# neo-sonar/neo-dsp

Hardware: AMD Instinct MI355X
Metric: Msamples/sec UPOLS convolver (block=512, IR=10s@48k); achieved HBM GB/s (higher is better)
Workload: dtype f32; 1 GPU; UPOLS c5full: 2048 channels in all, 2048 on rank 0 of 1 GPU(s) (split over the ranks), B=512, L=480000 taps (P=938), one block per step; channels_per_gpu=2048, channels_total=2048, block=512, taps=480000, partitions=938, far_group=3, step_group=4, far_form=transform, stored spectra, parallelism=channel-shard x1 (no collective)

## Files before the change

### neo-dsp_amd/csrc/upols_levels.hip

```cpp
#include "upols_device.hpp"
#include "upols_handle.hpp"

#include <algorithm>
#include <chrono>
#include <cmath>
#include <cstring>
#include <type_traits>
#include <vector>

namespace neo_hip {

#ifdef NEO_TIMELINE
#define NEO_TL_MARK(a)                                                                                 \
    do {                                                                                               \
        if (threadIdx.x == 0 && (a).tl)                                                                \
            static_cast<unsigned long long*>((a).tl)[4 * int64_t(blockIdx.x) + 3] = wall_clock64();    \
    } while (0)
#else
#define NEO_TL_MARK(a) \
    do {               \
    } while (0)
#endif
#ifdef NEO_PS_PROBE
#define NEO_PS_MARK(a, i)                                                                              \
// ... 282 lines not shown
        cmac(yb, h0b, xb, false);
        X[k0] = k0 == 0 ? c2r_join_w<B>(cf{ya.x, 0.f}, cf{ya.y, 0.f}, cf{1.f, 0.f}, 0)
                        : c2r_join_w<B>(ya, yb, cf{wa.x, -wa.y}, k0);
        X[k1] = c2r_join_w<B>(yb, k0 == 0 ? yb : ya, cf{wb.x, -wb.y}, k1);
    }
    __syncthreads();
    NEO_PS_MARK(a, 4);
    if (tid < 64) c2r_tail<B, OLA, EW, true, true, WT>(X, fft, tw, a.out + int64_t(c) * a.ld_out, prev_c, tid);
    NEO_PS_MARK(a, 5);
}

__device__ __forceinline__ __amdgpu_buffer_rsrc_t buf_rsrc(const void* p, int64_t bytes)
{
    return __builtin_amdgcn_make_buffer_rsrc(const_cast<void*>(p), 0, int(bytes), 0x00020000);
}

__device__ __forceinline__ cf buf_ld(__amdgpu_buffer_rsrc_t r, int voff, int soff)
{
    return __builtin_bit_cast(cf, __builtin_amdgcn_raw_buffer_load_b64(r, voff, soff, 2 ));
}

__device__ __forceinline__ void buf_st(cf v, __amdgpu_buffer_rsrc_t r, int voff, int soff)
{
    typedef unsigned u2v __attribute__((ext_vector_type(2)));
    __builtin_amdgcn_raw_buffer_store_b64(__builtin_bit_cast(u2v, v), r, voff, soff, 0);
}

#ifndef NEO_H_POLICY
#define NEO_H_POLICY 0
#endif
__device__ __forceinline__ cf ld_h(const cf* p, int band_end)
{
    if (NEO_H_POLICY && band_end <= 64) return *p;
    return ld_nt(p);
}

template<int D>
__device__ __forceinline__ float xor_sum(float v)
{
    const unsigned u = __float_as_uint(v);
    if constexpr (D == 16) {
        const auto r = __builtin_amdgcn_permlane16_swap(u, u, false, false);
        return __uint_as_float(r[0]) + __uint_as_float(r[1]);
    } else {
        static_assert(D == 32, "lane distance 16 or 32");
        const auto r = __builtin_amdgcn_permlane32_swap(u, u, false, false);
        return __uint_as_float(r[0]) + __uint_as_float(r[1]);
    }
}

template<int T, int NPL, int NPG, int JH>
__device__ __forceinline__ void toep_role(const slice_args& sa, const toep_arg& ta, int bid, char* smem)
{
    static_assert((NPG == 1 || NPG == 4 || NPG == 8 || NPG == 16) && T % JH == 0, "toeplitz slice geometry");
    constexpr int TJ = T / JH, LPU = 16 * NPG, UPW = 256 / LPU, WPU = NPG < 4 ? 1 : NPG / 4, NX = NPL + TJ - 1;
    f2v* red = reinterpret_cast<f2v*>(smem);
    const int t = threadIdx.x, col = t & 15, pg = (t >> 4) % NPG, us = t / LPU;
    const int wu = pg >> 2, q4 = pg & 3;
    const int gpc = sa.B / 16;
    int wb = bid;
    if constexpr (JH == 2 && UPW == 1) {
        if (bid < ta.nwg / 16 * 16) {
            const int r = bid & 15;
            wb = (bid & ~15) + (r & 7) * 2 + (r >> 3);
        }
    }
    const int u = ta.u0 + wb * UPW + us;
    const bool live = u < ta.u1;
    const int uc = live ? u : ta.u1 - 1;
    const int jh = uc % JH, cg = uc / JH, c = cg / gpc, k = (cg - c * gpc) * 16 + col;
    const int j0 = jh * TJ, pa = ta.a + pg * NPL;
    f2v acc[TJ];
#pragma unroll
    for (int j = 0; j < TJ; ++j) acc[j] = f2v(0.f);
    if constexpr (UPW == 1) {
        const int cu = __builtin_amdgcn_readfirstlane(c);
        const int ps8 = int(sa.pstride * int(sizeof(cf)));
        const __amdgpu_buffer_rsrc_t hres = buf_rsrc(sa.H + int64_t(cu) * sa.cstride, int64_t(ta.b) * ps8);
        const __amdgpu_buffer_rsrc_t xres = buf_rsrc(sa.fdl + int64_t(cu) * sa.cstride, int64_t(sa.ring) * ps8);
        if (live && pa < ta.b) {
            cf xr[NX], hm[NPL];
            int r0 = ta.tw + j0 + TJ - 1 - pa - (NX - 1);
            r0 = r0 < 0 ? r0 + sa.ring : r0;
            const int dw = sa.ring - r0;
            const int v0 = r0 * ps8 + k * int(sizeof(cf)), vw = v0 - sa.ring * ps8;
#pragma unroll
            for (int i = 0; i < NX; ++i) {
                const int d = NX - 1 - i;
                xr[i] = buf_ld(xres, (d >= dw ? vw : v0) + d * ps8, 0);
            }
            const int hv0 = pa * ps8 + k * int(sizeof(cf));
#pragma unroll
            for (int m = 0; m < NPL; ++m) hm[m] = buf_ld(hres, hv0, m * ps8);
#pragma unroll
            for (int m = 0; m < NPL; ++m) {
                const pk_coef h(hm[m], k == 0);
#pragma unroll
                for (int jj = 0; jj < TJ; ++jj) h.mac(acc[jj], xr[TJ - 1 - jj + m]);
            }
        }
    } else {
        const cf* Hc = sa.H + int64_t(c) * sa.cstride + k;
        const cf* Xc = sa.fdl + int64_t(c) * sa.cstride + k;
        if (live && pa < ta.b) {
            cf xr[NX], hm[NPL];
#pragma unroll
            for (int i = 0; i < NX; ++i) {
                int r = ta.tw + j0 + TJ - 1 - pa - i;
                r = r < 0 ? r + sa.ring : r;
                xr[i] = ld_nt(Xc + int64_t(r) * sa.pstride);
            }
#pragma unroll
            for (int m = 0; m < NPL; ++m) hm[m] = pa + m < ta.b ? ld_h(Hc + int64_t(pa + m) * sa.pstride, ta.b) : cf{0.f, 0.f};
#pragma unroll
            for (int m = 0; m < NPL; ++m) {
                const pk_coef h(hm[m], k == 0);
#pragma unroll
                for (int jj = 0; jj < TJ; ++jj) h.mac(acc[jj], xr[TJ - 1 - jj + m]);
            }
        }
    }
    if constexpr (NPG >= 4) {
#pragma unroll
        for (int j = 0; j < TJ; ++j) {
            acc[j].x = xor_sum<16>(acc[j].x);
            acc[j].y = xor_sum<16>(acc[j].y);
            acc[j].x = xor_sum<32>(acc[j].x);
            acc[j].y = xor_sum<32>(acc[j].y);
        }
    }
    if constexpr (WPU > 1) {
        if (wu > 0 && q4 == 0) {
#pragma unroll
            for (int j = 0; j < TJ; ++j) red[((us * (WPU - 1) + wu - 1) * TJ + j) * 16 + col] = acc[j];
        }
        __syncthreads();
    }
    if (wu == 0 && q4 == 0 && live) {
        cf* o = ta.slab + int64_t(c) * ta.cs + int64_t(j0) * sa.B + k;
#pragma unroll
        for (int j = 0; j < TJ; ++j) {
            f2v v = acc[j];
            if constexpr (WPU > 1) {
#pragma unroll
                for (int w = 1; w < WPU; ++w) v += red[((us * (WPU - 1) + w - 1) * TJ + j) * 16 + col];
            }
            o[int64_t(j) * sa.B] = cf{v.x, v.y};
        }
    }
}

__device__ __forceinline__ void cmac_pk(f2v& acc, cf h, cf x)
{
    const f2v xv = {x.x, x.y};
    acc = __builtin_elementwise_fma(f2v{h.x, h.x}, xv, acc);
    acc = __builtin_elementwise_fma(f2v{-h.y, h.y}, xv.yx, acc);
}

template<bool BIN0>
__device__ __forceinline__ void t32_step(f2v (&acc)[4], cf (&xw)[4], cf h, cf xn, bool z0)
{
    xw[3] = xw[2];
    xw[2] = xw[1];
    xw[1] = xw[0];
    xw[0] = xn;
    if constexpr (BIN0) {
        const pk_coef hk(h, z0);
#pragma unroll
        for (int o = 0; o < 4; ++o) hk.mac(acc[o], xw[o]);
    } else {
#pragma unroll
        for (int o = 0; o < 4; ++o) cmac_pk(acc[o], h, xw[o]);
    }
}

template<bool BIN0>
__device__ __forceinline__ void t32_walk(const cf* hc, const cf* xc, int ib, int m0, int m1, bool z0, f2v (&acc)[4])
{
    constexpr int KP = 4;
    cf xw[4];
#pragma unroll
    for (int o = 0; o < 3; ++o) xw[o] = xc[ib - m0 + 1 + o];
    int m = m0;
    for (; m + 2 * KP <= m1; m += 2 * KP) {
        float4 h2[KP], x2[KP];
#pragma unroll
        for (int i = 0; i < KP; ++i) {
            h2[i] = *reinterpret_cast<const float4*>(hc + m + 2 * i);
            x2[i] = *reinterpret_cast<const float4*>(xc + ib - (m + 2 * i) - 1);
        }
#pragma unroll
        for (int i = 0; i < KP; ++i) {
            t32_step<BIN0>(acc, xw, cf{h2[i].x, h2[i].y}, cf{x2[i].z, x2[i].w}, z0);
            t32_step<BIN0>(acc, xw, cf{h2[i].z, h2[i].w}, cf{x2[i].x, x2[i].y}, z0);
        }
    }
    for (; m < m1; ++m) t32_step<BIN0>(acc, xw, hc[m], xc[ib - m], z0);
}

template<int T, int NB, int JH>
struct toep_tile {
    static constexpr int UPW = 32 / T, LPU = 256 / UPW, NQ = LPU / 16;
    static constexpr int TP = T / JH, QUADS = TP / 4, NG = NQ / QUADS;
    static constexpr int HS = NB + 2, XS = NB + TP + 2;
    static constexpr int NH = (NB + NQ - 1) / NQ, NXL = (NB + TP - 1 + NQ - 1) / NQ;
    static constexpr int LDS = UPW * 16 * (HS + XS) * int(sizeof(cf));
    static_assert(NG >= 2 && NQ % QUADS == 0 && TP % 4 == 0, "toeplitz tile geometry");
};

template<int T, int NB, int JH>
__device__ __forceinline__ void toep_lds_role(const slice_args& sa, const toep_arg& ta, int bid, char* smem)
{
    using G = toep_tile<T, NB, JH>;
    static_assert(G::LDS <= kSliceLds, "toeplitz tile");
    const int t = threadIdx.x, us = t / G::LPU, lt = t % G::LPU, col = lt & 15, q = lt >> 4;
    cf* hs = reinterpret_cast<cf*>(smem) + us * 16 * (G::HS + G::XS);
    cf* xs = hs + 16 * G::HS;
    const int u = ta.u0 + bid * G::UPW + us, gpc = sa.B / 16;
    const bool live = u < ta.u1;
    const int uc = live ? u : ta.u1 - 1, jp = uc % JH, cg = uc / JH, c = cg / gpc, g = cg - c * gpc;
    const int k = g * 16 + col, nb = ta.b - ta.a, nx = nb + G::TP - 1, R = sa.ring, jpart = jp * G::TP;
    int rb = ta.tw + jpart - (ta.b - 1);
    rb = rb < 0 ? rb + R : rb;
    cf hv[G::NH], xv[G::NXL];
    if constexpr (G::UPW == 1) {
        const int cu = __builtin_amdgcn_readfirstlane(c), ps8 = int(sa.pstride * int(sizeof(cf)));
        const __amdgpu_buffer_rsrc_t hres = buf_rsrc(sa.H + int64_t(cu) * sa.cstride, int64_t(ta.b) * ps8);
        const __amdgpu_buffer_rsrc_t xres = buf_rsrc(sa.fdl + int64_t(cu) * sa.cstride, int64_t(R) * ps8);
#pragma unroll
        for (int i = 0; i < G::NH; ++i) {
            const int m = q + G::NQ * i;
            if (m < nb) hv[i] = buf_ld(hres, (ta.a + m) * ps8 + k * int(sizeof(cf)), 0);
        }
#pragma unroll
        for (int i = 0; i < G::NXL; ++i) {
            const int r = q + G::NQ * i;
            if (r < nx) xv[i] = buf_ld(xres, (rb + r >= R ? rb + r - R : rb + r) * ps8 + k * int(sizeof(cf)), 0);
        }
    } else {
        const cf* Hc = sa.H + int64_t(c) * sa.cstride + k;
        const cf* Xc = sa.fdl + int64_t(c) * sa.cstride + k;
#pragma unroll
        for (int i = 0; i < G::NH; ++i) {
            const int m = q + G::NQ * i;
            if (live && m < nb) hv[i] = ld_h(Hc + int64_t(ta.a + m) * sa.pstride, ta.b);
        }
#pragma unroll
        for (int i = 0; i < G::NXL; ++i) {
            const int r = q + G::NQ * i;
            if (live && r < nx) xv[i] = ld_nt(Xc + int64_t(rb + r >= R ? rb + r - R : rb + r) * sa.pstride);
        }
    }
    const int odd = nb & 1;
    if (live) {
#pragma unroll
        for (int i = 0; i < G::NH; ++i)
            if (q + G::NQ * i < nb) hs[col * G::HS + q + G::NQ * i] = hv[i];
#pragma unroll
        for (int i = 0; i < G::NXL; ++i)
            if (q + G::NQ * i < nx) xs[col * G::XS + odd + q + G::NQ * i] = xv[i];
    }
    __syncthreads();
    NEO_TL_MARK(sa);
    const int grp = q / G::QUADS, j0 = 4 * (q - grp * G::QUADS), nq = ((nb + G::NG - 1) / G::NG + 1) & ~1;
    const int m0 = grp * nq < nb ? grp * nq : nb, m1 = m0 + nq < nb ? m0 + nq : nb;
    f2v acc[4] = {f2v(0.f), f2v(0.f), f2v(0.f), f2v(0.f)};
    const cf* hc = hs + col * G::HS;
    const cf* xc = xs + col * G::XS + odd;
    if (live && m0 < m1) {
        if (g == 0) t32_walk<true>(hc, xc, j0 + nb - 1, m0, m1, col == 0, acc);
        else t32_walk<false>(hc, xc, j0 + nb - 1, m0, m1, false, acc);
    }
    __syncthreads();
    constexpr int LG = 16 * G::QUADS;
    f2v* red = reinterpret_cast<f2v*>(smem);
    const int lg = lt - grp * LG;
    if (grp) {
#pragma unroll
        for (int o = 0; o < 4; ++o) red[((us * (G::NG - 1) + grp - 1) * LG + lg) * 4 + o] = acc[o];
    }
    __syncthreads();
    if (!grp && live) {
        cf* o = ta.slab + int64_t(c) * ta.cs + int64_t(jpart + j0) * sa.B + k;
#pragma unroll
        for (int i = 0; i < 4; ++i) {
            f2v v = acc[i];
#pragma unroll
            for (int r = 1; r < G::NG; ++r) v += red[((us * (G::NG - 1) + r - 1) * LG + lg) * 4 + i];
            o[int64_t(i) * sa.B] = cf{v.x, v.y};
        }
    }
}

constexpr int kBigJH = 8, kBigJP = kBigT / kBigJH, kBigNC = 192;
constexpr int kBigHS = kBigNC + 2, kBigXS = kBigNC + kBigJP + 2;
static_assert(16 * (kBigHS + kBigXS) * int(sizeof(cf)) <= kSliceLds, "big level tile");

__device__ __forceinline__ void toep_big_role(const slice_args& sa, const toep_arg& ta, int bid, char* smem)
{
    constexpr int NH = kBigNC / 16, NXL = (kBigNC + kBigJP - 1 + 15) / 16;
    cf* hs = reinterpret_cast<cf*>(smem);
    cf* xs = hs + 16 * kBigHS;
    const int t = threadIdx.x, col = t & 15, qq = t >> 4, quad = qq & 3, quarter = qq >> 2;
    int wb = bid;
    if (bid < ta.nwg / 64 * 64) {
        const int r = bid & 63;
        wb = (bid & ~63) + (r & 7) * 8 + (r >> 3);
    }
    const int u = ta.u0 + wb, jp = u % kBigJH, cg = u / kBigJH, gpc = sa.B / 16;
    const int c = __builtin_amdgcn_readfirstlane(cg / gpc), g = __builtin_amdgcn_readfirstlane(cg - (cg / gpc) * gpc);
    const int k = g * 16 + col, nb = ta.b - ta.a, R = sa.ring, jpart = jp * kBigJP;
    const int ps8 = int(sa.pstride * int(sizeof(cf)));
    const __amdgpu_buffer_rsrc_t hres = buf_rsrc(sa.H + int64_t(c) * sa.cstride, int64_t(ta.b) * ps8);
    const __amdgpu_buffer_rsrc_t xres = buf_rsrc(sa.fdl + int64_t(c) * sa.cstride, int64_t(R) * ps8);
    f2v acc[4] = {f2v(0.f), f2v(0.f), f2v(0.f), f2v(0.f)};
    for (int mc = 0; mc < nb; mc += kBigNC) {
        const int nc = nb - mc < kBigNC ? nb - mc : kBigNC, nx = nc + kBigJP - 1;
        int rb = (ta.tw + jpart - (ta.a + mc + nc - 1)) % R;
        rb = rb < 0 ? rb + R : rb;
        cf hv[NH], xv[NXL];
#pragma unroll
        for (int i = 0; i < NH; ++i) {
            const int m = qq + 16 * i;
            if (m < nc) hv[i] = buf_ld(hres, (ta.a + mc + m) * ps8 + k * int(sizeof(cf)), 0);
        }
#pragma unroll
        for (int i = 0; i < NXL; ++i) {
            const int r = qq + 16 * i;
            if (r < nx) xv[i] = buf_ld(xres, (rb + r >= R ? rb + r - R : rb + r) * ps8 + k * int(sizeof(cf)), 0);
        }
        if (mc) __syncthreads();
        const int odd = nc & 1;
#pragma unroll
        for (int i = 0; i < NH; ++i)
            if (qq + 16 * i < nc) hs[col * kBigHS + qq + 16 * i] = hv[i];
#pragma unroll
        for (int i = 0; i < NXL; ++i)
            if (qq + 16 * i < nx) xs[col * kBigXS + odd + qq + 16 * i] = xv[i];
        __syncthreads();
        const int nq = ((nc + 3) / 4 + 1) & ~1, m0 = quarter * nq, m1 = m0 + nq < nc ? m0 + nq : nc;
        if (m0 < m1) {
            const cf* hc = hs + col * kBigHS;
            const cf* xc = xs + col * kBigXS + odd;
            if (g == 0) t32_walk<true>(hc, xc, nc - 1 + 4 * quad, m0, m1, col == 0, acc);
            else t32_walk<false>(hc, xc, nc - 1 + 4 * quad, m0, m1, false, acc);
        }
    }
    __syncthreads();
    f2v* red = reinterpret_cast<f2v*>(smem);
    const int ql = t & 63;
    if (quarter) {
#pragma unroll
        for (int o = 0; o < 4; ++o) red[((quarter - 1) * 64 + ql) * 4 + o] = acc[o];
    }
    __syncthreads();
    if (!quarter) {
        cf* o = ta.slab + int64_t(c) * ta.cs + int64_t(jpart + 4 * quad) * sa.B + k;
#pragma unroll
        for (int i = 0; i < 4; ++i) {
            const f2v v = acc[i] + red[ql * 4 + i] + red[(64 + ql) * 4 + i] + red[(128 + ql) * 4 + i];
            o[int64_t(i) * sa.B] = cf{v.x, v.y};
        }
    }
}


__device__ __forceinline__ cf pack_bin0(cf zf, cf zm, int f)
{
    if (f == 0 || f == kFN / 2) return zf;
    if (f < kFN / 2) return cscale(cadd(zf, cconj(zm)), 0.5f);
    const cf d = csub(zm, cconj(zf));
    return cf{0.5f * d.y, -0.5f * d.x};
}

__device__ __forceinline__ cf unpack_bin0(cf wf, cf wm, int f)
{
    if (f == 0 || f == kFN / 2) return wf;
    const cf dc = f < kFN / 2 ? wf : cconj(wm);
    const cf ny = f < kFN / 2 ? wm : cconj(wf);
    return cf{dc.x - ny.y, dc.y + ny.x};
}

template<bool PACK>
__device__ __forceinline__ void bin0_exchange(cf (&v)[16], cf* z, int a, int cp)
{
    if (cp == 0) {
#pragma unroll
        for (int i = 0; i < 16; ++i) z[a + 16 * i] = v[i];
    }
    __syncthreads();
    if (cp == 0) {
#pragma unroll
        for (int i = 0; i < 16; ++i) {
            const int f = a + 16 * i;
            const cf m = z[(kFN - f) & (kFN - 1)];
            v[i] = PACK ? pack_bin0(v[i], m, f) : unpack_bin0(v[i], m, f);
        }
    }
}

constexpr int kF1UG = 4;
constexpr int kFarKMax = 4;

__host__ __device__ __forceinline__ int far_first(int c, int K) { return 1 + ((c - 1) % K + K) % K; }

template<int FPL, int K>
__device__ __forceinline__ void far1_mac(const slice_args& sa, int u, int f0, int col)
{
    constexpr int NS = 16 / FPL;
    static_assert(NS >= K - 1 || K == 1, "history of the previous round");
    const int gpc = sa.B / 16, c = u / gpc, g = u - c * gpc, k = g * 16 + col;
    const int M = sa.M, nseg = sa.nseg, wn = sa.f1wn;
    auto slot = [&](int s) { return ((wn - s - 1) % M + M) % M; };
    const int64_t fs = sa.B, sp = int64_t(kFN) * fs;
    const int s0 = sa.fnfresh < nseg ? sa.fnfresh : nseg;
    const cf* hc = sa.hf + int64_t(c) * sa.fsc + int64_t(f0) * fs + k;
    const cf* xc = sa.xf + int64_t(c) * sa.fsc + int64_t(f0) * fs + k;
    f2v acc[K][FPL];
    cf xp[K > 1 ? K - 1 : 1][FPL];
    bool z0[FPL];
#pragma unroll
    for (int j = 0; j < FPL; ++j) {
#pragma unroll
        for (int w = 0; w < K; ++w) acc[w][j] = f2v(0.f);
        z0[j] = g == 0 && col == 0 && ((f0 + 4 * j) & (kFN / 2 - 1)) == 0;
    }
    for (int sb = s0; sb < nseg; sb += NS) {
        cf xv[NS][FPL], hv[NS][FPL];
#pragma unroll
        for (int i = 0; i < NS; ++i) {
            if (sb + i < nseg) {
                const cf* hs = hc + (sb + i) * sp;
                const cf* xs = xc + slot(sb + i) * sp;
#pragma unroll
                for (int j = 0; j < FPL; ++j) {
                    hv[i][j] = ld_nt(hs + 4 * j * fs);
                    xv[i][j] = ld_nt(xs + 4 * j * fs);
                }
            }
        }
#pragma unroll
        for (int i = 0; i < NS; ++i) {
            if (sb + i < nseg) {
#pragma unroll
                for (int j = 0; j < FPL; ++j) {
                    const pk_coef h(hv[i][j], z0[j]);
#pragma unroll
                    for (int w = 0; w < K; ++w)
                        if (sb + i - w >= s0) h.mac(acc[w][j], i >= w ? xv[i - w][j] : xp[w - i - 1][j]);
                }
            }
        }
        if constexpr (K > 1) {
#pragma unroll
            for (int d = 0; d < K - 1; ++d)
#pragma unroll
                for (int j = 0; j < FPL; ++j) xp[d][j] = xv[NS - 1 - d][j];
        }
    }
#pragma unroll
    for (int w = 0; w < K; ++w) {
        cf* o = sa.f1acc + (int64_t(((wn + w) % sa.fK) * sa.fU + u) * kFN + f0) * 16 + col;
#pragma unroll
        for (int j = 0; j < FPL; ++j) o[4 * j * 16] = cf{acc[w][j].x, acc[w][j].y};
    }
}

template<int FPL, int KMAX>
__device__ __forceinline__ void far1_role(const slice_args& sa, int bid)
{
    constexpr int FR = 4 * FPL, PPG = kFN / FR;
    const int t = threadIdx.x, cl = t & 63, fq = t >> 6;
    const int grp = bid / PPG, part = bid - grp * PPG;
    const int g4 = sa.f1g0 + grp * sa.f1gs;
    const int u = g4 * kF1UG + (cl >> 4);
    if (u < sa.f1u0 || u >= sa.f1u1) return;
    const int f0 = part * FR + fq;
    const int K = sa.fK, cls = sa.f1mode ? g4 % K : 0;
    if (sa.f1mode == 0 || (cls != sa.f1cls && far_first(cls, K) > sa.f1wn)) {
        far1_mac<FPL, 1>(sa, u, f0, cl & 15);
    } else if (cls == sa.f1cls) {
        if constexpr (KMAX <= 2) {
            far1_mac<FPL, 2>(sa, u, f0, cl & 15);
        } else {
            if (K == 2) far1_mac<FPL, 2>(sa, u, f0, cl & 15);
            else if (K == 3) far1_mac<FPL, 3>(sa, u, f0, cl & 15);
            else far1_mac<FPL, kFarKMax>(sa, u, f0, cl & 15);
        }
    }
}

__device__ __forceinline__ void far2a_role(const slice_args& sa, int bid, char* smem)
{
    cf* lds = reinterpret_cast<cf*>(smem);
    cf* z = lds + 16 * 16 * 16;
    cf* tws = z + kFN;
    const int t = threadIdx.x, a = t >> 4, cp = t & 15;
    const int gpc = sa.B / 16, u = sa.f2u0 + bid, c = u / gpc, g = u - c * gpc, k = g * 16 + cp;
// ... 230 lines not shown
        if (unit0) bin0_exchange<true>(hv, z, a, cp);
#pragma unroll
        for (int i = 0; i < 16; ++i) pk_coef(hv[i], z0(i)).mac(acc[i], x[i]);
    }
    cf v[16];
#pragma unroll
    for (int i = 0; i < 16; ++i) v[i] = cf{acc[i].x, acc[i].y};
    __syncthreads();
    NEO_TL_MARK(sa);
    if (unit0) bin0_exchange<false>(v, z, a, cp);
    col_fft<1, 16>(v, lds, tws, a, cp, true);
    constexpr float sc = 1.0f / kFN;
    const __amdgpu_buffer_rsrc_t ores = buf_rsrc(sa.f3ff + int64_t(c) * sa.fcs, int(kFN * fs * int(sizeof(cf))) / 2);
    const int vo = int((int64_t(a) * fs + k) * int(sizeof(cf)));
#pragma unroll
    for (int m = 8; m < 16; ++m)
        buf_st(cscale(v[m], sc), ores, vo, int(16 * (m - 8) * fs * int(sizeof(cf))));
}

struct off_args {
    const cf* fdl;
    const cf* hf;
    const cf* twf;
    cf* y;
    int64_t cstride, pstride;
    int64_t hcs;
    int ring, B, nseg, w;
};

#ifndef NEO_OFF_PF
#define NEO_OFF_PF 0
#endif
template<int WP>
__global__ __launch_bounds__(256) __attribute__((amdgpu_waves_per_eu(WP == 1 ? 3 : 2))) void k_off_mac(off_args sa)
{
    __shared__ cf lds[16 * 16 * 16];
    __shared__ cf z[kFN];
    __shared__ cf tws[kFN];
    __shared__ cf xh[8 * 256];
    const int t = threadIdx.x, a = t >> 4, cp = t & 15;
    const int gpc = sa.B / 16, u = blockIdx.x, c = u / gpc, g = u - c * gpc, k = g * 16 + cp;
    const bool unit0 = g == 0;
    const int64_t fs = sa.B;
    const int spec = int(int64_t(kFN) * fs * int(sizeof(cf)));
    tws[t] = sa.twf[t];
    const __amdgpu_buffer_rsrc_t fres =
        buf_rsrc(sa.fdl + int64_t(c) * sa.cstride, int64_t(sa.ring) * sa.pstride * int(sizeof(cf)));
    const __amdgpu_buffer_rsrc_t hres = buf_rsrc(sa.hf + int64_t(c) * sa.hcs, int64_t(sa.nseg) * spec);
    const int ps8 = int(sa.pstride * int(sizeof(cf))), ko = k * int(sizeof(cf));
    const int vo = int((int64_t(a) * fs + k) * int(sizeof(cf)));
    auto z0 = [&](int i) { return unit0 && cp == 0 && ((a + 16 * i) & (kFN / 2 - 1)) == 0; };
    auto row = [&](int r) { return r >= sa.ring ? r - sa.ring : r; };
    f2v acc[WP][16];
#pragma unroll
    for (int w = 0; w < WP; ++w)
#pragma unroll
        for (int i = 0; i < 16; ++i) acc[w][i] = f2v(0.f);
    int r0 = (sa.w + kFarT * (WP - 2) + a) % sa.ring;
    r0 = r0 < 0 ? r0 + sa.ring : r0;
    cf xp[WP > 1 ? 16 : 1];
    cf nx[NEO_OFF_PF >= 1 ? 8 : 1], nh[NEO_OFF_PF >= 2 ? 16 : 1];
    auto load_rows = [&](cf* dst, int n0, int n1) {
#pragma unroll
        for (int n = n0; n < n1; ++n) dst[n - n0] = buf_ld(fres, row(r0 + 16 * n) * ps8 + ko, 0);
    };
    auto load_spec = [&](cf* dst, int q) {
#pragma unroll
        for (int i = 0; i < 16; ++i) dst[i] = buf_ld(hres, vo, q * spec + int(16 * i * fs * int(sizeof(cf))));
    };
    __syncthreads();
    for (int q = 1 - WP; q < sa.nseg; ++q) {
        cf x[16], hv[16];
        if (q == 1 - WP) {
            load_rows(x, 0, 16);
        } else {
            if constexpr (NEO_OFF_PF >= 1) {
#pragma unroll
                for (int n = 0; n < 8; ++n) x[n] = nx[n];
            } else {
                load_rows(x, 0, 8);
            }
#pragma unroll
            for (int n = 8; n < 16; ++n) x[n] = xh[(n - 8) * 256 + t];
        }
        if (q >= 0) {
            if constexpr (NEO_OFF_PF >= 2) {
                if (q == 0) load_spec(hv, 0);
                else {
#pragma unroll
                    for (int i = 0; i < 16; ++i) hv[i] = nh[i];
                }
            } else {
                load_spec(hv, q);
            }
        }
#pragma unroll
        for (int n = 0; n < 8; ++n) xh[n * 256 + t] = x[n];
        r0 = r0 - kFarT < 0 ? r0 - kFarT + sa.ring : r0 - kFarT;
        if constexpr (NEO_OFF_PF >= 1)
            if (q + 1 < sa.nseg) load_rows(nx, 0, 8);
        if constexpr (NEO_OFF_PF >= 2)
            if (q + 1 < sa.nseg && q + 1 >= 1) load_spec(nh, q + 1);
        col_fft<-1, 16>(x, lds, tws, a, cp, true);
        if (unit0) bin0_exchange<true>(x, z, a, cp);
        if (q >= 0) {
#pragma unroll
            for (int i = 0; i < 16; ++i) {
                const pk_coef h(hv[i], z0(i));
                h.mac(acc[0][i], x[i]);
                if constexpr (WP > 1) h.mac(acc[1][i], xp[i]);
            }
        }
        if constexpr (WP > 1) {
#pragma unroll
            for (int i = 0; i < 16; ++i) xp[i] = x[i];
        }
    }
    constexpr float sc = 1.0f / kFN;
#pragma unroll
    for (int w = 0; w < WP; ++w) {
        cf v[16];
#pragma unroll
        for (int i = 0; i < 16; ++i) v[i] = cf{acc[w][i].x, acc[w][i].y};
        __syncthreads();
        if (unit0) bin0_exchange<false>(v, z, a, cp);
        col_fft<1, 16>(v, lds, tws, a, cp, true);
        const __amdgpu_buffer_rsrc_t ores =
            buf_rsrc(sa.y + (int64_t(c) * WP + w) * kFarT * fs, int64_t(kFarT) * fs * int(sizeof(cf)));
#pragma unroll
        for (int m = 8; m < 16; ++m)
            buf_st(cscale(v[m], sc), ores, vo, int(16 * (m - 8) * fs * int(sizeof(cf))));
    }
}

#ifndef NEO_ROLES
#define NEO_ROLES 63
#endif

template<int L>
__device__ __forceinline__ bool toep_level(const slice_args& a, int& bid, char* smem)
{
    if (L >= a.ntp) return false;
    const toep_arg ta = a.tp[L];
    if (bid >= ta.nwg) {
        bid -= ta.nwg;
        return false;
    }
    static_assert(kLvT0 == 4 && kLvToep == 5, "level slots: windows 4, 8, 16, 32 (bands 2T, 2T, 2T, 6T), 128");
    if constexpr (L == 0) {
        if (NEO_ROLES & 2) toep_role<4, 8, 1, 1>(a, ta, bid, smem);
    } else if constexpr (L == 1) {
        if (NEO_ROLES & 2) toep_role<8, 16, 1, 1>(a, ta, bid, smem);
    } else if constexpr (L == 2) {
        if (NEO_ROLES & 2) toep_lds_role<16, 32, 1>(a, ta, bid, smem);
    } else if constexpr (L == 3) {
        if (NEO_ROLES & 4) {
            if (ta.jh == 2) toep_lds_role<32, kT32Band, 2>(a, ta, bid, smem);
            else toep_lds_role<32, kT32Band, 1>(a, ta, bid, smem);
        }
    } else {
        if (NEO_ROLES & 4) toep_big_role(a, ta, bid, smem);
    }
    return true;
}

template<int L>
__device__ __forceinline__ bool toep_skip(const slice_args& a, int& bid)
{
    if (L >= a.ntp) return false;
    if (bid >= a.tp[L].nwg) {
        bid -= a.tp[L].nwg;
        return false;
    }
    return true;
}

#ifndef NEO_STEP_WPE
#define NEO_STEP_WPE 3
#endif
#ifndef NEO_RAW_WPE
#define NEO_RAW_WPE 2
#endif
template<int KMAX>
constexpr int slices_wpe() { return KMAX == 1 ? NEO_RAW_WPE : NEO_STEP_WPE; }
template<int B, int KMAX = 2>
constexpr int step_wpe() { return B > 512 ? 2 : (KMAX == 1 ? NEO_RAW_WPE : NEO_STEP_WPE); }
#ifndef NEO_ORDER
#define NEO_ORDER 0
#endif
template<int B, bool OLA, int KMAX, int PART = 0>
__device__ __forceinline__ int lvl_roles(const slice_args& a, char* smem)
{
    int bid = int(blockIdx.x) + a.bid0;
    auto far2b = [&]() {
        if (bid >= a.f3nwg) {
            bid -= a.f3nwg;
            return false;
        }
        if ((NEO_ROLES & 32) && threadIdx.x < 256) {
            if constexpr (KMAX == 1) far2r_role(a, bid, smem);
            else if (a.f2comb) far2c_role<KMAX>(a, bid, smem);
            else far2b_role<KMAX>(a, bid, smem);
        }
        return true;
    };
    auto far2a = [&]() {
        if (bid >= a.f2nwg) {
            bid -= a.f2nwg;
            return false;
        }
        if constexpr (KMAX > 1)
            if ((NEO_ROLES & 16) && threadIdx.x < 256) far2a_role(a, bid, smem);
        return true;
    };
    auto block = [&]() {
        if constexpr (PART == 2) return false;
        if (bid >= a.nblk) {
            bid -= a.nblk;
            return false;
        }
        if (NEO_ROLES & 1) block_role<B, OLA>(a, a.blk_c0 + bid, smem);
        return true;
    };
    if constexpr (PART == 1) {
        if (block()) return 3;
        if (threadIdx.x >= 256) return 0;
        if (toep_level<0>(a, bid, smem)) return 4;
        return toep_level<1>(a, bid, smem) ? 5 : 0;
    }
    auto far1 = [&]() {
        if (bid >= a.f1nwg) {
            bid -= a.f1nwg;
            return false;
        }
        if constexpr (KMAX > 1) {
            if ((NEO_ROLES & 8) && threadIdx.x < 256) {
                if (a.f1fpl == 4) far1_role<4, KMAX>(a, bid);
                else if (a.f1fpl == 2) far1_role<2, KMAX>(a, bid);
                else far1_role<1, KMAX>(a, bid);
            }
        }
        return true;
    };
    auto toep = [&](auto L) { return threadIdx.x < 256 ? toep_level<decltype(L)::value>(a, bid, smem)
                                                       : toep_skip<decltype(L)::value>(a, bid); };
    using L0 = std::integral_constant<int, 0>;
    using L1 = std::integral_constant<int, 1>;
    using L2 = std::integral_constant<int, 2>;
    using L3 = std::integral_constant<int, 3>;
    using L4 = std::integral_constant<int, 4>;
#if NEO_ORDER == 2
    if (toep(L4{})) return 8;
    if (toep(L3{})) return 7;
#endif
    if (far2b()) return 1;
    if (far2a()) return 2;
    if (block()) return 3;
#if NEO_ORDER == 3
    {
        int A = 0;
#pragma unroll
        for (int l = 0; l < kLvToep; ++l)
            if (l < a.ntp) A += a.tp[l].nwg;
        const int F = a.f1nwg, N = A + F;
        if (F > 0 && bid < N) {
            const int f0 = int(int64_t(bid) * F / N), f1 = int(int64_t(bid + 1) * F / N);
            if (f1 > f0) {
                bid = f0 + A;
            } else {
                bid -= f0;
            }
        }
    }
#endif
#if NEO_ORDER != 2
    if (toep(L4{})) return 8;
    if (toep(L3{})) return 7;
#endif
#if NEO_ORDER == 1
    if (far1()) return 9;
#endif
    if (toep(L2{})) return 6;
    if (toep(L1{})) return 5;
    if (toep(L0{})) return 4;
#if NEO_ORDER != 1
    if (far1()) return 9;
#endif
    return 0;
}

template<int B>
constexpr int block_lds() { return (B + upols_cfg<B>::LL + upols_cfg<B>::TW1 + upols_cfg<B>::TW2) * int(sizeof(cf)); }

#ifndef NEO_BLOCK_PRIO
#define NEO_BLOCK_PRIO 0
#endif
#ifndef NEO_BLOCK_WPE
#define NEO_BLOCK_WPE 1
#endif
#ifdef NEO_TIMELINE
template<int WG, class F>
__device__ __forceinline__ void tl_record(const slice_args& a, F roles)
{
    const unsigned long long t0 = wall_clock64();
    const int role = roles();
    if constexpr (WG > 256) return;
    __syncthreads();
    if (threadIdx.x == 0 && a.tl) {
        unsigned long long* r = static_cast<unsigned long long*>(a.tl) + 4 * int64_t(blockIdx.x);
        r[0] = t0;
        r[1] = wall_clock64();
// ... 1446 lines not shown
```

Baseline: 9527 Msamples/s.

## Widen T32 Toeplitz lanes to eight outputs with software-pipelined LDS reads

The T=32 level Toeplitz tile now computes eight outputs per lane instead of four. Each coefficient/input pair loaded from LDS is reused across more accumulators, and the walk loop double-buffers its reads with sched barriers. The complex MAC is hand-written as v_pk_fma_f32 inline asm with op_sel/neg modifiers, and quad indices are swizzled by column to avoid LDS bank conflicts. The reduction now spreads the final sums across all groups instead of group 0 only. This trades higher register pressure and fewer parallel groups for less LDS traffic per FMA.

```diff
diff --git a/neo-dsp_amd/csrc/upols_levels.hip b/neo-dsp_amd/csrc/upols_levels.hip
--- a/neo-dsp_amd/csrc/upols_levels.hip
+++ b/neo-dsp_amd/csrc/upols_levels.hip
@@ -458,66 +458,117 @@
 
 __device__ __forceinline__ void cmac_pk(f2v& acc, cf h, cf x)
 {
-    const f2v xv = {x.x, x.y};
-    acc = __builtin_elementwise_fma(f2v{h.x, h.x}, xv, acc);
-    acc = __builtin_elementwise_fma(f2v{-h.y, h.y}, xv.yx, acc);
-}
-
-template<bool BIN0>
-__device__ __forceinline__ void t32_step(f2v (&acc)[4], cf (&xw)[4], cf h, cf xn, bool z0)
-{
-    xw[3] = xw[2];
-    xw[2] = xw[1];
-    xw[1] = xw[0];
+    const f2v hv = {h.x, h.y}, xv = {x.x, x.y};
+    asm("v_pk_fma_f32 %0, %1, %2, %0 op_sel_hi:[0,1,1]" : "+v"(acc) : "v"(hv), "v"(xv));
+    asm("v_pk_fma_f32 %0, %1, %2, %0 op_sel:[1,1,0] op_sel_hi:[1,0,1] neg_lo:[1,0,0]" : "+v"(acc) : "v"(hv), "v"(xv));
+}
+
+template<bool BIN0, int NO>
+__device__ __forceinline__ void t32_step(f2v (&acc)[NO], cf (&xw)[NO], cf h, cf xn, bool z0)
+{
+#pragma unroll
+    for (int o = NO - 1; o > 0; --o) xw[o] = xw[o - 1];
     xw[0] = xn;
     if constexpr (BIN0) {
         const pk_coef hk(h, z0);
 #pragma unroll
-        for (int o = 0; o < 4; ++o) hk.mac(acc[o], xw[o]);
+        for (int o = 0; o < NO; ++o) hk.mac(acc[o], xw[o]);
     } else {
 #pragma unroll
-        for (int o = 0; o < 4; ++o) cmac_pk(acc[o], h, xw[o]);
-    }
-}
-
-template<bool BIN0>
-__device__ __forceinline__ void t32_walk(const cf* hc, const cf* xc, int ib, int m0, int m1, bool z0, f2v (&acc)[4])
-{
-    constexpr int KP = 4;
-    cf xw[4];
-#pragma unroll
-    for (int o = 0; o < 3; ++o) xw[o] = xc[ib - m0 + 1 + o];
+        for (int o = 0; o < NO; ++o) cmac_pk(acc[o], h, xw[o]);
+    }
+}
+
+template<bool BIN0, int NO>
+__device__ __forceinline__ void t32_walk(const cf* hc, const cf* xc, int ib, int m0, int m1, bool z0, f2v (&acc)[NO])
+{
+    static_assert(NO == 4 || NO == 8, "outputs per lane");
+    cf xw[NO];
+#pragma unroll
+    for (int o = 0; o < NO - 1; ++o) xw[o] = xc[ib - m0 + 1 + o];
     int m = m0;
-    for (; m + 2 * KP <= m1; m += 2 * KP) {
-        float4 h2[KP], x2[KP];
-#pragma unroll
-        for (int i = 0; i < KP; ++i) {
-            h2[i] = *reinterpret_cast<const float4*>(hc + m + 2 * i);
-            x2[i] = *reinterpret_cast<const float4*>(xc + ib - (m + 2 * i) - 1);
-        }
-#pragma unroll
-        for (int i = 0; i < KP; ++i) {
-            t32_step<BIN0>(acc, xw, cf{h2[i].x, h2[i].y}, cf{x2[i].z, x2[i].w}, z0);
-            t32_step<BIN0>(acc, xw, cf{h2[i].z, h2[i].w}, cf{x2[i].x, x2[i].y}, z0);
-        }
-    }
-    for (; m < m1; ++m) t32_step<BIN0>(acc, xw, hc[m], xc[ib - m], z0);
-}
-
-template<int T, int NB, int JH>
+    if constexpr (NO == 4) {
+        constexpr int KP = 4;
+        for (; m + 2 * KP <= m1; m += 2 * KP) {
+            float4 h2[KP], x2[KP];
+#pragma unroll
+            for (int i = 0; i < KP; ++i) {
+                h2[i] = *reinterpret_cast<const float4*>(hc + m + 2 * i);
+                x2[i] = *reinterpret_cast<const float4*>(xc + ib - (m + 2 * i) - 1);
+            }
+#pragma unroll
+            for (int i = 0; i < KP; ++i) {
+                t32_step<BIN0, NO>(acc, xw, cf{h2[i].x, h2[i].y}, cf{x2[i].z, x2[i].w}, z0);
+                t32_step<BIN0, NO>(acc, xw, cf{h2[i].z, h2[i].w}, cf{x2[i].x, x2[i].y}, z0);
+            }
+        }
+    } else {
+        constexpr int KP = 2;
+        const int n = (m1 - m0) / (4 * KP);
+        if (n > 0) {
+            const int ml = m0 + (n - 1) * 4 * KP;
+            float4 ha[KP], xa[KP], hb[KP], xb[KP];
+            const auto rd = [&](float4 (&h2)[KP], float4 (&x2)[KP], int mm) {
+#pragma unroll
+                for (int i = 0; i < KP; ++i) {
+                    h2[i] = *reinterpret_cast<const float4*>(hc + mm + 2 * i);
+                    x2[i] = *reinterpret_cast<const float4*>(xc + ib - (mm + 2 * i) - 1);
+                }
+            };
+            const auto go = [&](const float4 (&h2)[KP], const float4 (&x2)[KP]) {
+#pragma unroll
+                for (int i = 0; i < KP; ++i) {
+                    t32_step<BIN0, NO>(acc, xw, cf{h2[i].x, h2[i].y}, cf{x2[i].z, x2[i].w}, z0);
+                    t32_step<BIN0, NO>(acc, xw, cf{h2[i].z, h2[i].w}, cf{x2[i].x, x2[i].y}, z0);
+                }
+            };
+            const auto two = [&](int mm) {
+                rd(hb, xb, mm + 2 * KP);
+                __builtin_amdgcn_sched_barrier(0);
+                go(ha, xa);
+                __builtin_amdgcn_sched_barrier(0);
+                rd(ha, xa, mm + 4 * KP < ml ? mm + 4 * KP : ml);
+                __builtin_amdgcn_sched_barrier(0);
+                go(hb, xb);
+                __builtin_amdgcn_sched_barrier(0);
+            };
+            rd(ha, xa, m);
+            int it = 0;
+            for (; it + 2 <= n; it += 2, m += 8 * KP) {
+                two(m);
+                two(m + 4 * KP);
+            }
+            if (it < n) {
+                two(m);
+                m += 4 * KP;
+            }
+        }
+        for (; m + 2 <= m1; m += 2) {
+            const float4 h2 = *reinterpret_cast<const float4*>(hc + m);
+            const float4 x2 = *reinterpret_cast<const float4*>(xc + ib - m - 1);
+            t32_step<BIN0, NO>(acc, xw, cf{h2.x, h2.y}, cf{x2.z, x2.w}, z0);
+            t32_step<BIN0, NO>(acc, xw, cf{h2.z, h2.w}, cf{x2.x, x2.y}, z0);
+        }
+    }
+    for (; m < m1; ++m) t32_step<BIN0, NO>(acc, xw, hc[m], xc[ib - m], z0);
+}
+
+template<int T, int NB, int JH, int NO>
 struct toep_tile {
     static constexpr int UPW = 32 / T, LPU = 256 / UPW, NQ = LPU / 16;
-    static constexpr int TP = T / JH, QUADS = TP / 4, NG = NQ / QUADS;
+    static constexpr int TP = T / JH, PARTS = TP / NO, NG = NQ / PARTS;
     static constexpr int HS = NB + 2, XS = NB + TP + 2;
     static constexpr int NH = (NB + NQ - 1) / NQ, NXL = (NB + TP - 1 + NQ - 1) / NQ;
     static constexpr int LDS = UPW * 16 * (HS + XS) * int(sizeof(cf));
-    static_assert(NG >= 2 && NQ % QUADS == 0 && TP % 4 == 0, "toeplitz tile geometry");
+    static_assert(NG >= 2 && NQ % PARTS == 0 && TP % NO == 0 && NQ % 2 == 0, "toeplitz tile geometry");
+    static_assert(HS / 2 % 2 == 1 && XS / 2 % 2 == 1, "odd column strides in 16-B units: conflict-free pair reads");
+    static_assert(UPW * NG * 16 * PARTS * NO * int(sizeof(f2v)) <= LDS, "the groups' partial sums fit the freed tile");
 };
 
-template<int T, int NB, int JH>
+template<int T, int NB, int JH, int NO>
 __device__ __forceinline__ void toep_lds_role(const slice_args& sa, const toep_arg& ta, int bid, char* smem)
 {
-    using G = toep_tile<T, NB, JH>;
+    using G = toep_tile<T, NB, JH, NO>;
     static_assert(G::LDS <= kSliceLds, "toeplitz tile");
     const int t = threadIdx.x, us = t / G::LPU, lt = t % G::LPU, col = lt & 15, q = lt >> 4;
     cf* hs = reinterpret_cast<cf*>(smem) + us * 16 * (G::HS + G::XS);
@@ -568,31 +619,34 @@
     }
     __syncthreads();
     NEO_TL_MARK(sa);
-    const int grp = q / G::QUADS, j0 = 4 * (q - grp * G::QUADS), nq = ((nb + G::NG - 1) / G::NG + 1) & ~1;
+    const int qw = q ^ (((col + 4) >> 3) & 1);
+    const int grp = qw / G::PARTS, part = qw - grp * G::PARTS, j0 = NO * part, nq = ((nb + G::NG - 1) / G::NG + 1) & ~1;
     const int m0 = grp * nq < nb ? grp * nq : nb, m1 = m0 + nq < nb ? m0 + nq : nb;
-    f2v acc[4] = {f2v(0.f), f2v(0.f), f2v(0.f), f2v(0.f)};
+    f2v acc[NO];
+#pragma unroll
+    for (int o = 0; o < NO; ++o) acc[o] = f2v(0.f);
     const cf* hc = hs + col * G::HS;
     const cf* xc = xs + col * G::XS + odd;
     if (live && m0 < m1) {
-        if (g == 0) t32_walk<true>(hc, xc, j0 + nb - 1, m0, m1, col == 0, acc);
-        else t32_walk<false>(hc, xc, j0 + nb - 1, m0, m1, false, acc);
+        if (g == 0) t32_walk<true, NO>(hc, xc, j0 + nb - 1, m0, m1, col == 0, acc);
+        else t32_walk<false, NO>(hc, xc, j0 + nb - 1, m0, m1, false, acc);
     }
     __syncthreads();
-    constexpr int LG = 16 * G::QUADS;
-    f2v* red = reinterpret_cast<f2v*>(smem);
-    const int lg = lt - grp * LG;
-    if (grp) {
-#pragma unroll
-        for (int o = 0; o < 4; ++o) red[((us * (G::NG - 1) + grp - 1) * LG + lg) * 4 + o] = acc[o];
-    }
+    constexpr int LG = 16 * G::PARTS, OPG = NO / G::NG;
+    static_assert(NO % G::NG == 0, "the groups share the sum");
+    f2v* red = reinterpret_cast<f2v*>(smem) + us * G::NG * NO * LG;
+    const int lg = part * 16 + col;
+#pragma unroll
+    for (int o = 0; o < NO; ++o) red[(grp * NO + o) * LG + lg] = acc[o];
     __syncthreads();
-    if (!grp && live) {
-        cf* o = ta.slab + int64_t(c) * ta.cs + int64_t(jpart + j0) * sa.B + k;
-#pragma unroll
-        for (int i = 0; i < 4; ++i) {
-            f2v v = acc[i];
-#pragma unroll
-            for (int r = 1; r < G::NG; ++r) v += red[((us * (G::NG - 1) + r - 1) * LG + lg) * 4 + i];
+    if (live) {
+        const int o0 = grp * OPG;
+        cf* o = ta.slab + int64_t(c) * ta.cs + int64_t(jpart + j0 + o0) * sa.B + k;
+#pragma unroll
+        for (int i = 0; i < OPG; ++i) {
+            f2v v = red[(o0 + i) * LG + lg];
+#pragma unroll
+            for (int r = 1; r < G::NG; ++r) v += red[(r * NO + o0 + i) * LG + lg];
             o[int64_t(i) * sa.B] = cf{v.x, v.y};
         }
     }
@@ -648,8 +702,8 @@
         if (m0 < m1) {
             const cf* hc = hs + col * kBigHS;
             const cf* xc = xs + col * kBigXS + odd;
-            if (g == 0) t32_walk<true>(hc, xc, nc - 1 + 4 * quad, m0, m1, col == 0, acc);
-            else t32_walk<false>(hc, xc, nc - 1 + 4 * quad, m0, m1, false, acc);
+            if (g == 0) t32_walk<true, 4>(hc, xc, nc - 1 + 4 * quad, m0, m1, col == 0, acc);
+            else t32_walk<false, 4>(hc, xc, nc - 1 + 4 * quad, m0, m1, false, acc);
         }
     }
     __syncthreads();
@@ -1186,11 +1240,11 @@
     } else if constexpr (L == 1) {
         if (NEO_ROLES & 2) toep_role<8, 16, 1, 1>(a, ta, bid, smem);
     } else if constexpr (L == 2) {
-        if (NEO_ROLES & 2) toep_lds_role<16, 32, 1>(a, ta, bid, smem);
+        if (NEO_ROLES & 2) toep_lds_role<16, 32, 1, 4>(a, ta, bid, smem);
     } else if constexpr (L == 3) {
         if (NEO_ROLES & 4) {
-            if (ta.jh == 2) toep_lds_role<32, kT32Band, 2>(a, ta, bid, smem);
-            else toep_lds_role<32, kT32Band, 1>(a, ta, bid, smem);
+            if (ta.jh == 2) toep_lds_role<32, kT32Band, 2, 8>(a, ta, bid, smem);
+            else toep_lds_role<32, kT32Band, 1, 8>(a, ta, bid, smem);
         }
     } else {
         if (NEO_ROLES & 4) toep_big_role(a, ta, bid, smem);
```

After: 9662 Msamples/s, median of 6. Within noise of the previous version (+1.4%).
